# uber/fiber

Hardware: AMD Instinct MI355X
Metric: es_rollouts_per_sec (higher is better)
Workload: dtype bf16; 1 GPU; model=es-mlp-obs4-h64x64-act2, global_batch=2097152, seq_len=256, parallelism=dp1, pop_per_gpu=32768, envs_per_member=64

## Files before the change

### fiber_amd/csrc/ops/bindings.cpp

```cpp

#include <hip/hip_bf16.h>
#include <hip/hip_runtime.h>
#include <pybind11/pybind11.h>
#include <rocprim/rocprim.hpp>

#include <stdexcept>
#include <string>

namespace py = pybind11;

#define NPARAMS_HOST 4610
#define ENVS_HOST 64
#define OBS_HOST 4

extern "C" __global__ void es_rollout_mlp(
    const float*, float, uint32_t, uint32_t, int, int, const float*,
    const float*, const float*, const float*, float*, float*, float*);
extern "C" __global__ void es_eval_matrix(const float*, const float*,
                                          const float*, const float*,
                                          const float*, uint32_t, uint32_t,
                                          int, int, float*, float*);
extern "C" __global__ void obs_stat_reduce(const float*, int, float*);
extern "C" __global__ void es_grad(const float*, int, int, int, uint32_t,
                                   uint32_t, int, float*);
extern "C" __global__ void es_grad_reduce(const float*, int, int, float*);
extern "C" __global__ void centered_rank(const float*, int, float*);
extern "C" __global__ void rank_pack_keys(const float*, int, unsigned*,
                                          unsigned*);
extern "C" __global__ void rank_scatter(const unsigned*, int, float*);
extern "C" __global__ void mlp_policy_forward(const float*, const float*,
                                              int, float*);
extern "C" __global__ void mfma_gemm64_probe(const float*, const float*,
                                             float*);
extern "C" __global__ void es_perturb(const float*, int, int, float,
                                      uint32_t, const uint32_t*, int,
                                      __hip_bfloat16*, unsigned char*,
                                      unsigned char*);
extern "C" __global__ void conv_env_init(uint32_t, const uint32_t*, int,
                                         float*, float*);
extern "C" __global__ void conv_noisegen(uint32_t, const uint32_t*,
                                         uint32_t, unsigned char*);
extern "C" __global__ void conv_layer1(const __hip_bfloat16*,
                                       const unsigned char*, const float*,
                                       const __hip_bfloat16*,
                                       const unsigned char*, int,
                                       __hip_bfloat16*);
extern "C" __global__ void conv_layer2(const __hip_bfloat16*,
                                       const __hip_bfloat16*, int,
                                       unsigned char*);
extern "C" __global__ void conv_fc(const __hip_bfloat16*,
                                   const unsigned char*,
                                   const unsigned char*, int,
                                   __hip_bfloat16*);
extern "C" __global__ void conv_head_env(const __hip_bfloat16*,
                                         const __hip_bfloat16*, int,
                                         const float*, const float*, float*,
                                         float*);

static void check(hipError_t err, const char* what) {
  if (err != hipSuccess) {
    throw std::runtime_error(std::string(what) + ": " +
                             hipGetErrorString(err));
  }
}

static void launch_rollout(uintptr_t theta, double sigma, uint32_t seed,
                           uint32_t iter, int horizon, int member_offset,
                           int pop_shard, uintptr_t obs_mu, uintptr_t obs_nu,
                           uintptr_t env_A, uintptr_t env_B,
                           uintptr_t fitness, uintptr_t obs_stat_part,
                           uintptr_t obs_stat, uintptr_t stream) {
  if (pop_shard <= 0) return;
  hipLaunchKernelGGL(es_rollout_mlp, dim3(pop_shard), dim3(256), 0,
                     (hipStream_t)stream, (const float*)theta, (float)sigma,
                     seed, iter, horizon, member_offset,
                     (const float*)obs_mu, (const float*)obs_nu,
                     (const float*)env_A, (const float*)env_B,
                     (float*)fitness, (float*)obs_stat_part,
                     (float*)obs_stat);
  check(hipGetLastError(), "es_rollout_mlp launch");
  hipLaunchKernelGGL(obs_stat_reduce, dim3(2 * OBS_HOST), dim3(256), 0,
                     (hipStream_t)stream, (const float*)obs_stat_part,
                     pop_shard, (float*)obs_stat);
  check(hipGetLastError(), "obs_stat_reduce launch");
}

static void launch_eval_matrix(uintptr_t thetas, uintptr_t obs_mu,
                               uintptr_t obs_nu, uintptr_t env_A,
                               uintptr_t env_B, uint32_t seed, uint32_t iter,
                               int horizon, int K, int M, uintptr_t scores,
                               uintptr_t episodes, uintptr_t stream) {
  if (K <= 0 || M <= 0) return;
  const long long cells = (long long)K * (long long)M;
  if (cells > 0x7FFFFFFFLL)
    throw std::runtime_error("es_eval_matrix: K*M exceeds the grid limit");
  if (horizon < 1)
    throw std::runtime_error("es_eval_matrix: horizon must be >= 1");
  hipLaunchKernelGGL(es_eval_matrix, dim3((unsigned)cells), dim3(256), 0,
                     (hipStream_t)stream, (const float*)thetas,
                     (const float*)obs_mu, (const float*)obs_nu,
                     (const float*)env_A, (const float*)env_B, seed, iter,
                     horizon, M, (float*)scores, (float*)episodes);
  check(hipGetLastError(), "es_eval_matrix launch");
}

static int grad_chunks(int pairs, int nparams) {
  const int bx = ((nparams + 3) / 4 + 255) / 256;
  return pairs < 64 ? 1 : (bx >= 32 ? 4 : 32);
}

static void launch_grad(uintptr_t wpair, int pair_begin, int pair_end,
                        uint32_t seed, uint32_t iter, int nparams,
                        uintptr_t grad_part, uintptr_t grad,
                        uintptr_t stream) {
  const int jblocks = (nparams + 3) / 4;
  const int bx = (jblocks + 255) / 256;
  int pairs = pair_end - pair_begin;
  if (pairs <= 0) return;
  const int chunks = grad_chunks(pairs, nparams);
  int per_chunk = (pairs + chunks - 1) / chunks;
  hipLaunchKernelGGL(es_grad, dim3(bx, chunks), dim3(256), 0,
                     (hipStream_t)stream, (const float*)wpair, pair_begin,
                     pair_end, per_chunk, seed, iter, nparams,
                     chunks == 1 ? (float*)grad : (float*)grad_part);
  check(hipGetLastError(), "es_grad launch");
  if (chunks > 1) {
    hipLaunchKernelGGL(es_grad_reduce, dim3((nparams + 255) / 256),
                       dim3(256), 0, (hipStream_t)stream,
                       (const float*)grad_part, chunks, nparams,
                       (float*)grad);
    check(hipGetLastError(), "es_grad_reduce launch");
  }
}

static void launch_centered_rank(uintptr_t f, int n, uintptr_t out,
                                 uintptr_t stream) {
  const int bx = (n + 255) / 256;
  hipLaunchKernelGGL(centered_rank, dim3(bx), dim3(256), 0,
                     (hipStream_t)stream, (const float*)f, n, (float*)out);
  check(hipGetLastError(), "centered_rank launch");
}

static inline uint64_t rank_array_stride(int n) {
  return (((uint64_t)n * 4) + 255) & ~(uint64_t)255;
}

static uint64_t centered_rank_sorted_workspace(int n) {
  size_t temp_bytes = 0;
  check(rocprim::radix_sort_pairs(nullptr, temp_bytes,
                                  (const unsigned*)nullptr,
                                  (unsigned*)nullptr,
                                  (const unsigned*)nullptr,
                                  (unsigned*)nullptr, (size_t)n),
        "radix_sort_pairs size query");
  return 4 * rank_array_stride(n) + (uint64_t)temp_bytes + 256;
}

static void launch_centered_rank_sorted(uintptr_t f, int n, uintptr_t out,
                                        uintptr_t work, uint64_t work_bytes,
                                        uintptr_t stream) {
  const uint64_t stride = rank_array_stride(n);
  if (work_bytes < 4 * stride)
    throw std::runtime_error("centered_rank_sorted workspace too small");
  unsigned* keys_in = (unsigned*)work;
  unsigned* keys_out = (unsigned*)(work + stride);
  unsigned* vals_in = (unsigned*)(work + 2 * stride);
  unsigned* vals_out = (unsigned*)(work + 3 * stride);
  void* temp = (void*)(work + 4 * stride);
  size_t temp_bytes = (size_t)(work_bytes - 4 * stride);
  const int bx = (n + 255) / 256;
  hipLaunchKernelGGL(rank_pack_keys, dim3(bx), dim3(256), 0,
                     (hipStream_t)stream, (const float*)f, n, keys_in,
                     vals_in);
  check(hipGetLastError(), "rank_pack_keys launch");
  check(rocprim::radix_sort_pairs(temp, temp_bytes, keys_in, keys_out,
                                  vals_in, vals_out, (size_t)n, 0, 32,
                                  (hipStream_t)stream),
        "radix_sort_pairs");
  hipLaunchKernelGGL(rank_scatter, dim3(bx), dim3(256), 0,
                     (hipStream_t)stream, vals_out, n, (float*)out);
  check(hipGetLastError(), "rank_scatter launch");
}

static void launch_mlp_forward(uintptr_t theta, uintptr_t x, int batch,
                               uintptr_t logits, uintptr_t stream) {
  const int bx = (batch + ENVS_HOST - 1) / ENVS_HOST;
  hipLaunchKernelGGL(mlp_policy_forward, dim3(bx), dim3(256), 0,
                     (hipStream_t)stream, (const float*)theta,
                     (const float*)x, batch, (float*)logits);
  check(hipGetLastError(), "mlp_policy_forward launch");
}

static void launch_gemm64_probe(uintptr_t a, uintptr_t b, uintptr_t c,
                                uintptr_t stream) {
  hipLaunchKernelGGL(mfma_gemm64_probe, dim3(1), dim3(256), 0,
                     (hipStream_t)stream, (const float*)a, (const float*)b,
                     (float*)c);
  check(hipGetLastError(), "mfma_gemm64_probe launch");
}


static void launch_perturb(uintptr_t theta, int nparams, int np_pad,
                           double sigma, uint32_t seed, uintptr_t iterp,
                           int member_offset, int pop, uintptr_t wpert,
                           uintptr_t w3_fp8, uintptr_t w1_fp8,
                           uintptr_t stream) {
  if ((member_offset | pop) & 1)
    throw std::runtime_error(
        "es_perturb needs pair-aligned member_offset/pop");
  const int bx = 64;
  hipLaunchKernelGGL(es_perturb, dim3(bx, pop / 2), dim3(256), 0,
                     (hipStream_t)stream, (const float*)theta, nparams,
                     np_pad, (float)sigma, seed, (const uint32_t*)iterp,
                     member_offset, (__hip_bfloat16*)wpert,
                     (unsigned char*)w3_fp8, (unsigned char*)w1_fp8);
  check(hipGetLastError(), "es_perturb launch");
}

static void launch_conv_env_init(uint32_t seed, uintptr_t iterp,
                                 int nmembers, uintptr_t state,
                                 uintptr_t racc, uintptr_t stream) {
  const int n = nmembers * 16;
  hipLaunchKernelGGL(conv_env_init, dim3((n + 255) / 256), dim3(256), 0,
                     (hipStream_t)stream, seed, (const uint32_t*)iterp,
                     nmembers, (float*)state, (float*)racc);
  check(hipGetLastError(), "conv_env_init launch");
}

static void launch_conv_noisegen(uint32_t seed, uintptr_t iterp, uint32_t t,
                                 int nenv, uintptr_t znoise,
                                 uintptr_t stream) {
  const int total = nenv * (84 * 84 / 4);
  hipLaunchKernelGGL(conv_noisegen, dim3((total + 255) / 256), dim3(256), 0,
                     (hipStream_t)stream, seed, (const uint32_t*)iterp, t,
                     (unsigned char*)znoise);
  check(hipGetLastError(), "conv_noisegen launch");
}

static void launch_conv_layer1(uintptr_t wpert, uintptr_t w1_fp8,
                               uintptr_t state, uintptr_t gtab,
                               uintptr_t znoise, uintptr_t act1,
                               int nmembers, uintptr_t stream) {
  const int nenv = nmembers * 16;
  hipLaunchKernelGGL(conv_layer1, dim3(nenv), dim3(256), 0,
                     (hipStream_t)stream, (const __hip_bfloat16*)wpert,
                     (const unsigned char*)w1_fp8, (const float*)state,
                     (const __hip_bfloat16*)gtab,
                     (const unsigned char*)znoise, nenv,
                     (__hip_bfloat16*)act1);
  check(hipGetLastError(), "conv_layer1 launch");
}

static void launch_conv_layer2(uintptr_t wpert, uintptr_t act1,
                               uintptr_t act2, int nmembers,
                               uintptr_t stream) {
  const int nenv = nmembers * 16;
  hipLaunchKernelGGL(conv_layer2, dim3(nenv), dim3(256), 0,
                     (hipStream_t)stream, (const __hip_bfloat16*)wpert,
                     (const __hip_bfloat16*)act1, nenv,
                     (unsigned char*)act2);
  check(hipGetLastError(), "conv_layer2 launch");
}

static void launch_conv_fc(uintptr_t wpert, uintptr_t w3_fp8,
                           uintptr_t act2, uintptr_t act3, int nmembers,
                           uintptr_t stream) {
  hipLaunchKernelGGL(conv_fc, dim3(nmembers, 4), dim3(256), 0,
                     (hipStream_t)stream, (const __hip_bfloat16*)wpert,
                     (const unsigned char*)w3_fp8,
                     (const unsigned char*)act2, nmembers,
                     (__hip_bfloat16*)act3);
  check(hipGetLastError(), "conv_fc launch");
}

static void launch_conv_forward(uintptr_t wpert, uintptr_t w3_fp8,
                                uintptr_t w1_fp8, uintptr_t state,
                                uintptr_t gtab, uintptr_t znoise,
                                uintptr_t act1, uintptr_t act2,
                                uintptr_t act3, int nmembers,
                                uintptr_t stream) {
  launch_conv_layer1(wpert, w1_fp8, state, gtab, znoise, act1, nmembers,
                     stream);
  launch_conv_layer2(wpert, act1, act2, nmembers, stream);
  launch_conv_fc(wpert, w3_fp8, act2, act3, nmembers, stream);
}

static void launch_conv_head_env(uintptr_t wpert, uintptr_t act3,
                                 int nmembers, uintptr_t env_A,
                                 uintptr_t env_B, uintptr_t state,
                                 uintptr_t racc, uintptr_t stream) {
  hipLaunchKernelGGL(conv_head_env, dim3(nmembers), dim3(256), 0,
                     (hipStream_t)stream, (const __hip_bfloat16*)wpert,
                     (const __hip_bfloat16*)act3, nmembers,
                     (const float*)env_A, (const float*)env_B,
                     (float*)state, (float*)racc);
  check(hipGetLastError(), "conv_head_env launch");
}

PYBIND11_MODULE(_ops, m) {
  m.doc() = "fiber_amd CDNA4 ES kernels (gfx950)";
  m.attr("NPARAMS") = NPARAMS_HOST;
  m.attr("ENVS_PER_MEMBER") = ENVS_HOST;
  m.def("es_rollout_mlp", &launch_rollout, py::arg("theta"),
        py::arg("sigma"), py::arg("seed"), py::arg("iter"),
        py::arg("horizon"), py::arg("member_offset"), py::arg("pop_shard"),
        py::arg("obs_mu"), py::arg("obs_nu"), py::arg("env_A"),
        py::arg("env_B"), py::arg("fitness"), py::arg("obs_stat_part"),
        py::arg("obs_stat"), py::arg("stream"));
  m.def("es_eval_matrix", &launch_eval_matrix, py::arg("thetas"),
        py::arg("obs_mu"), py::arg("obs_nu"), py::arg("env_A"),
        py::arg("env_B"), py::arg("seed"), py::arg("iter"),
        py::arg("horizon"), py::arg("K"), py::arg("M"), py::arg("scores"),
        py::arg("episodes"), py::arg("stream"));
  m.def("es_grad", &launch_grad, py::arg("wpair"), py::arg("pair_begin"),
        py::arg("pair_end"), py::arg("seed"), py::arg("iter"),
        py::arg("nparams"), py::arg("grad_part"), py::arg("grad"),
        py::arg("stream"));
  m.def("es_grad_chunks", &grad_chunks, py::arg("pairs"),
        py::arg("nparams"));
  m.def("centered_rank", &launch_centered_rank, py::arg("f"), py::arg("n"),
        py::arg("out"), py::arg("stream"));
  m.def("centered_rank_sorted_workspace", &centered_rank_sorted_workspace,
        py::arg("n"));
  m.def("centered_rank_sorted", &launch_centered_rank_sorted, py::arg("f"),
        py::arg("n"), py::arg("out"), py::arg("work"),
        py::arg("work_bytes"), py::arg("stream"));
  m.def("mlp_policy_forward", &launch_mlp_forward, py::arg("theta"),
        py::arg("x"), py::arg("batch"), py::arg("logits"),
        py::arg("stream"));
  m.def("mfma_gemm64_probe", &launch_gemm64_probe, py::arg("a"),
        py::arg("b"), py::arg("c"), py::arg("stream"));

  m.attr("NP_CONV") = 677686;
  m.attr("NP_CONV_PAD") = 677688;
  m.attr("CONV_ENVS") = 16;
  m.def("es_perturb", &launch_perturb, py::arg("theta"), py::arg("nparams"),
        py::arg("np_pad"), py::arg("sigma"), py::arg("seed"),
        py::arg("iterp"), py::arg("member_offset"), py::arg("pop"),
        py::arg("wpert"), py::arg("w3_fp8"), py::arg("w1_fp8"),
        py::arg("stream"));
  m.def("conv_env_init", &launch_conv_env_init, py::arg("seed"),
        py::arg("iterp"), py::arg("nmembers"), py::arg("state"),
        py::arg("racc"), py::arg("stream"));
  m.def("conv_noisegen", &launch_conv_noisegen, py::arg("seed"),
        py::arg("iterp"), py::arg("t"), py::arg("nenv"),
        py::arg("znoise"), py::arg("stream"));
  m.def("conv_forward", &launch_conv_forward, py::arg("wpert"),
        py::arg("w3_fp8"), py::arg("w1_fp8"), py::arg("state"),
        py::arg("gtab"), py::arg("znoise"), py::arg("act1"),
        py::arg("act2"), py::arg("act3"), py::arg("nmembers"),
        py::arg("stream"));
  m.def("conv_layer1", &launch_conv_layer1, py::arg("wpert"),
        py::arg("w1_fp8"), py::arg("state"), py::arg("gtab"),
        py::arg("znoise"), py::arg("act1"), py::arg("nmembers"),
        py::arg("stream"));
  m.def("conv_layer2", &launch_conv_layer2, py::arg("wpert"),
        py::arg("act1"), py::arg("act2"), py::arg("nmembers"),
        py::arg("stream"));
  m.def("conv_fc", &launch_conv_fc, py::arg("wpert"), py::arg("w3_fp8"),
        py::arg("act2"), py::arg("act3"), py::arg("nmembers"),
        py::arg("stream"));
  m.def("conv_head_env", &launch_conv_head_env, py::arg("wpert"),
        py::arg("act3"), py::arg("nmembers"), py::arg("env_A"),
        py::arg("env_B"), py::arg("state"), py::arg("racc"),
        py::arg("stream"));
}
```

### fiber_amd/csrc/ops/es_kernels.hip

```cpp

#include <hip/hip_bf16.h>
#include <hip/hip_runtime.h>

#include "philox.h"

typedef __attribute__((ext_vector_type(8))) __bf16 bf16x8;
typedef __attribute__((ext_vector_type(4))) float f32x4;
typedef __attribute__((ext_vector_type(2))) float f32x2;

#define TWO_LOG2E 0x1.715476p+1f
__device__ inline float fast_tanh(float x) {
  float e = __builtin_amdgcn_exp2f(x * TWO_LOG2E);
  return 1.0f - 2.0f * __builtin_amdgcn_rcpf(e + 1.0f);
}

__device__ inline f32x2 tanh2_bias(f32x2 acc, f32x2 bias) {
  const f32x2 m = (acc + bias) * TWO_LOG2E;
  f32x2 e;
  e.x = __builtin_amdgcn_exp2f(m.x);
  e.y = __builtin_amdgcn_exp2f(m.y);
  const f32x2 ep1 = e + 1.0f;
  f32x2 r;
  r.x = __builtin_amdgcn_rcpf(ep1.x);
  r.y = __builtin_amdgcn_rcpf(ep1.y);
  return __builtin_elementwise_fma(r, (f32x2){-2.0f, -2.0f},
                                   (f32x2){1.0f, 1.0f});
}

__device__ inline f32x4 fast_tanh4_bias(f32x4 acc, f32x4 bias) {
  const f32x2 lo = tanh2_bias(acc.lo, bias.lo);
  const f32x2 hi = tanh2_bias(acc.hi, bias.hi);
  return __builtin_shufflevector(lo, hi, 0, 1, 2, 3);
}

#define FAM_TAG_NOISE 0x45530001u
#define FAM_TAG_ENV 0x45530002u

#define OBS 4
#define KPAD 32
#define HID 64
#define ACT 2
#define ENVS 64

#define OFF_W1 0
#define OFF_B1 (HID * OBS)
#define OFF_W2 (OFF_B1 + HID)
#define OFF_B2 (OFF_W2 + HID * HID)
#define OFF_W3 (OFF_B2 + HID)
#define OFF_B3 (OFF_W3 + ACT * HID)
#define NPARAMS (OFF_B3 + ACT)

#define S1 8
#define S2 72

template <int S, bool NARROW>
__device__ inline const bf16x8* strip_frag_ptr(
    const __hip_bfloat16* __restrict__ M, const __hip_bfloat16* zero16,
    int row, int kk, int kgrp) {
  if (NARROW)
    return reinterpret_cast<const bf16x8*>(kgrp == 0 ? &M[row * S] : zero16);
  return reinterpret_cast<const bf16x8*>(&M[row * S + kk * 32 + kgrp * 8]);
}

template <int K, int AS, bool NARROW = false>
__device__ inline void strip_load_a(const __hip_bfloat16* __restrict__ A,
                                    const __hip_bfloat16* zero16, int wave,
                                    int lane, bf16x8 (&afrag)[K / 32]) {
#pragma unroll
  for (int kk = 0; kk < K / 32; ++kk)
    afrag[kk] = *strip_frag_ptr<AS, NARROW>(A, zero16,
                                            wave * 16 + (lane & 15), kk,
                                            lane >> 4);
}

__device__ inline f32x4 strip_load_bias(const float* __restrict__ bias,
                                        int wave, int lane) {
  return *reinterpret_cast<const f32x4*>(
      &bias[wave * 16 + (lane >> 4) * 4]);
}

template <int K, int BS, bool NARROW>
__device__ inline f32x4 strip_mfma(const bf16x8 (&afrag)[K / 32],
                                   const __hip_bfloat16* __restrict__ B,
                                   const __hip_bfloat16* zero16, int ct,
                                   int lane) {
  f32x4 acc = {0.f, 0.f, 0.f, 0.f};
#pragma unroll
  for (int kk = 0; kk < K / 32; ++kk) {
    const bf16x8 bfrag = *strip_frag_ptr<BS, NARROW>(
        B, zero16, ct * 16 + (lane & 15), kk, lane >> 4);
    acc = __builtin_amdgcn_mfma_f32_16x16x32_bf16(afrag[kk], bfrag, acc, 0,
                                                  0, 0);
  }
  return acc;
}

template <int K, int BS, int OS, bool NARROW = false>
__device__ inline void mfma_strip_tanh_pre(
    const bf16x8 (&afrag)[K / 32], const __hip_bfloat16* __restrict__ B,
    const __hip_bfloat16* zero16, f32x4 biasq,
    __hip_bfloat16* __restrict__ out, int wave, int lane) {
#pragma unroll
  for (int ct = 0; ct < 4; ++ct) {
    const int bcol = ct * 16 + (lane & 15);
    const f32x4 acc = strip_mfma<K, BS, NARROW>(afrag, B, zero16, ct, lane);
    const int drow = wave * 16 + (lane >> 4) * 4;
    const f32x4 th = fast_tanh4_bias(acc, biasq);
    union {
      __hip_bfloat16 h[4];
      unsigned long long u;
    } pk;
#pragma unroll
    for (int ri = 0; ri < 4; ++ri) pk.h[ri] = __float2bfloat16(th[ri]);
    *reinterpret_cast<unsigned long long*>(&out[bcol * OS + drow]) = pk.u;
  }
}

template <int K, int AS, int BS, int OS, bool NARROW = false>
__device__ inline void mfma_strip_tanh(const __hip_bfloat16* __restrict__ A,
                                       const __hip_bfloat16* __restrict__ B,
                                       const float* __restrict__ bias,
                                       __hip_bfloat16* __restrict__ out,
                                       int wave, int lane,
                                       const __hip_bfloat16* zero16 = nullptr) {
  bf16x8 afrag[K / 32];
  strip_load_a<K, AS, NARROW>(A, zero16, wave, lane, afrag);
  mfma_strip_tanh_pre<K, BS, OS, NARROW>(
      afrag, B, zero16, strip_load_bias(bias, wave, lane), out, wave, lane);
}

template <int K, int BS>
__device__ inline void mfma_strip_logits(
    const bf16x8 (&afrag)[K / 32], const __hip_bfloat16* __restrict__ B,
    f32x4 biasq, const float* __restrict__ w3r, float (*lpart)[ENVS][2],
    int wave, int lane) {
#pragma unroll
  for (int ct = 0; ct < 4; ++ct) {
    const f32x4 acc = strip_mfma<K, BS, false>(afrag, B, nullptr, ct, lane);
    const f32x4 h = fast_tanh4_bias(acc, biasq);
    float p0 = 0.f, p1 = 0.f;
#pragma unroll
    for (int ri = 0; ri < 4; ++ri) {
      p0 += w3r[ri] * h[ri];
      p1 += w3r[4 + ri] * h[ri];
    }
    p0 += __shfl_xor(p0, 16, 64);
    p1 += __shfl_xor(p1, 16, 64);
    p0 += __shfl_xor(p0, 32, 64);
    p1 += __shfl_xor(p1, 32, 64);
    if ((lane >> 4) == 0) {
      lpart[wave][ct * 16 + lane][0] = p0;
      lpart[wave][ct * 16 + lane][1] = p1;
    }
  }
}

struct PolicyLds {
  alignas(16) __hip_bfloat16 w1[HID][S1];
  alignas(16) __hip_bfloat16 w2[HID][S2];
  alignas(16) __hip_bfloat16 w3[ACT][HID];
  alignas(16) float b1[HID];
  alignas(16) float b2[HID];
  float b3[ACT];
};

__device__ inline void store_param(PolicyLds* p, int j, float v) {
  if (j < OFF_B1) {
    p->w1[j >> 2][j & 3] = __float2bfloat16(v);
  } else if (j < OFF_W2) {
    p->b1[j - OFF_B1] = v;
  } else if (j < OFF_B2) {
    int jj = j - OFF_W2;
    p->w2[jj >> 6][jj & 63] = __float2bfloat16(v);
  } else if (j < OFF_W3) {
    p->b2[j - OFF_B2] = v;
  } else if (j < OFF_B3) {
    int jj = j - OFF_W3;
    p->w3[jj >> 6][jj & 63] = __float2bfloat16(v);
  } else if (j < NPARAMS) {
    p->b3[j - OFF_B3] = v;
  }
}

struct RolloutLds {
  PolicyLds pol;
  alignas(16) __hip_bfloat16 xb[ENVS][S1];
  alignas(16) __hip_bfloat16 zero16[8];
  alignas(16) __hip_bfloat16 h1[ENVS][S2];
  float S[2][ENVS][OBS];
  float lpart[4][ENVS][2];
  float ostat[2 * OBS + 1];
};


template <bool STATS>
__device__ __forceinline__ void rollout_init_lds(RolloutLds& L, int tid,
                                                 uint32_t seed,
                                                 uint32_t iter) {
  for (int idx = tid; idx < HID * (S1 - OBS); idx += blockDim.x) {
    L.pol.w1[idx / (S1 - OBS)][OBS + idx % (S1 - OBS)] =
        __float2bfloat16(0.f);
  }
  for (int idx = tid; idx < ENVS * (S1 - OBS); idx += blockDim.x) {
    L.xb[idx / (S1 - OBS)][OBS + idx % (S1 - OBS)] =
        __float2bfloat16(0.f);
  }
  if (tid < 8) L.zero16[tid] = __float2bfloat16(0.f);
  if (tid < ENVS) {
    float z[4];
    fam_normal4(seed, iter, (uint32_t)tid, 0u, FAM_TAG_ENV, 0u, z);
#pragma unroll
    for (int d = 0; d < OBS; ++d) L.S[0][tid][d] = 0.3f * z[d];
  }
  if (STATS) {
    if (tid < 2 * OBS + 1) L.ostat[tid] = 0.f;
  }
}

template <bool STATS>
__device__ __forceinline__ float rollout_steps(
    RolloutLds& L, int tid, int horizon, const float* obs_mu,
    const float* obs_nu,
    const float* env_A,
    const float* env_B,
    float& psum, float& psq) {
  const int lane = tid & 63;
  const int wave = tid >> 6;
  const int env = tid & 63;
  const int dd = tid >> 6;
  float raccp = 0.f;
  const float mu_d = obs_mu[dd];
  const float rstd_d = rsqrtf(obs_nu[dd] + 1e-4f);
  float eA_d[OBS];
#pragma unroll
  for (int e = 0; e < OBS; ++e) eA_d[e] = env_A[dd * OBS + e];
  const float eB_d = env_B[dd];
  const float one_if_d0 = (dd == 0) ? 1.f : 0.f;
  float w3r[2 * 4];
  {
    const int drow = wave * 16 + (lane >> 4) * 4;
#pragma unroll
    for (int ri = 0; ri < 4; ++ri) {
      w3r[ri] = __bfloat162float(L.pol.w3[0][drow + ri]);
      w3r[4 + ri] = __bfloat162float(L.pol.w3[1][drow + ri]);
    }
  }

  bf16x8 a1[KPAD / 32], a2[HID / 32];
  strip_load_a<KPAD, S1, true>(&L.pol.w1[0][0], L.zero16, wave, lane, a1);
  strip_load_a<HID, S2>(&L.pol.w2[0][0], nullptr, wave, lane, a2);
  const f32x4 b1q = strip_load_bias(L.pol.b1, wave, lane);
  const f32x4 b2q = strip_load_bias(L.pol.b2, wave, lane);

  {
    const float s = L.S[0][env][dd];
    if (STATS) {
      psum += s;
      psq += s * s;
    }
    float x = (s - mu_d) * rstd_d;
    L.xb[env][dd] = __float2bfloat16(fminf(5.f, fmaxf(-5.f, x)));
  }

  for (int t = 0; t < horizon; ++t) {
    const int cur = t & 1;
    __syncthreads();
    mfma_strip_tanh_pre<KPAD, S1, S2, true>(a1, &L.xb[0][0], L.zero16, b1q,
                                            &L.h1[0][0], wave, lane);
    __syncthreads();
    mfma_strip_logits<HID, S2>(a2, &L.h1[0][0], b2q, w3r, L.lpart, wave,
                               lane);
    __syncthreads();
    {
      const float l0 = L.pol.b3[0] + L.lpart[0][env][0] +
                       L.lpart[1][env][0] + L.lpart[2][env][0] +
                       L.lpart[3][env][0];
      const float l1 = L.pol.b3[1] + L.lpart[0][env][1] +
                       L.lpart[1][env][1] + L.lpart[2][env][1] +
                       L.lpart[3][env][1];
      const float asign = (l1 > l0) ? 1.f : -1.f;
      float drive = 0.f;
#pragma unroll
      for (int e = 0; e < OBS; ++e) drive += eA_d[e] * L.S[cur][env][e];
      const float snew =
          fmaf(0.08f, fast_tanh(drive), 0.97f * L.S[cur][env][dd]) +
          0.05f * eB_d * asign;
      L.S[cur ^ 1][env][dd] = snew;
      raccp += one_if_d0 - 0.1f * snew * snew;
      if (t < horizon - 1) {
        if (STATS) {
          psum += snew;
          psq += snew * snew;
        }
        float x = (snew - mu_d) * rstd_d;
        L.xb[env][dd] = __float2bfloat16(fminf(5.f, fmaxf(-5.f, x)));
      }
    }
  }
  __syncthreads();
  return raccp;
}

__device__ __forceinline__ float reward_reduce_wave0(
    const RolloutLds& L, int lane, float* __restrict__ episodes) {
  float r = L.lpart[0][lane][0] + L.lpart[1][lane][0] +
            L.lpart[2][lane][0] + L.lpart[3][lane][0];
  if (episodes != nullptr) episodes[lane] = r;
#pragma unroll
  for (int off = 32; off > 0; off >>= 1) r += __shfl_down(r, off, 64);
  return r;
}

extern "C" __global__ void __launch_bounds__(256)
es_rollout_mlp(const float* __restrict__ theta, float sigma, uint32_t seed,
               uint32_t iter, int horizon, int member_offset,
               const float* __restrict__ obs_mu,
               const float* __restrict__ obs_nu,
               const float* __restrict__ env_A,
               const float* __restrict__ env_B,
               float* __restrict__ fitness,
               float* __restrict__ obs_stat_part,
               float* __restrict__ obs_stat_out)
{
  __shared__ RolloutLds L;
  const int tid = threadIdx.x;
  const int lane = tid & 63;
  const int wave = tid >> 6;
  const int member = member_offset + blockIdx.x;
  const uint32_t pair = (uint32_t)(member >> 1);
  const float sgn = (member & 1) ? -sigma : sigma;

  for (int jb = tid; jb * 4 < NPARAMS; jb += blockDim.x) {
    float z[4];
    fam_normal4(seed, iter, pair, (uint32_t)jb, FAM_TAG_NOISE, 0u, z);
    const int j0 = jb * 4;
#pragma unroll
    for (int u = 0; u < 4; ++u) {
      const int j = j0 + u;
      if (j < NPARAMS) store_param(&L.pol, j, theta[j] + sgn * z[u]);
    }
  }
  rollout_init_lds<true>(L, tid, seed, iter);
  __syncthreads();

  const int env = tid & 63;
  const int dd = tid >> 6;
  float psum = 0.f, psq = 0.f;
  const float raccp = rollout_steps<true>(L, tid, horizon, obs_mu, obs_nu,
                                          env_A, env_B, psum, psq);

  L.lpart[dd][env][0] = raccp;
#pragma unroll
  for (int off = 32; off > 0; off >>= 1) {
    psum += __shfl_down(psum, off, 64);
    psq += __shfl_down(psq, off, 64);
  }
  if (lane == 0) {
    L.ostat[dd] = psum;
    L.ostat[OBS + dd] = psq;
  }
  __syncthreads();
  if (wave == 0) {
    const float r = reward_reduce_wave0(L, lane, nullptr);
    if (lane == 0) fitness[blockIdx.x] = r / (float)ENVS;
  }
  if (tid < 2 * OBS)
    obs_stat_part[(size_t)blockIdx.x * (2 * OBS) + tid] = L.ostat[tid];
  if (tid == 0)
    atomicAdd(&obs_stat_out[2 * OBS], (float)(ENVS * horizon));
}

extern "C" __global__ void __launch_bounds__(256)
es_eval_matrix(const float* __restrict__ thetas,
               const float* __restrict__ obs_mu,
               const float* __restrict__ obs_nu,
               const float* __restrict__ env_A,
               const float* __restrict__ env_B,
               uint32_t seed, uint32_t iter, int horizon, int M,
               float* __restrict__ scores,
               float* __restrict__ episodes)
{
  __shared__ RolloutLds L;
  const int tid = threadIdx.x;
  const size_t cell = blockIdx.x;
  const size_t k = cell / (size_t)M;
  const size_t m = cell % (size_t)M;

  const float* __restrict__ theta = thetas + k * NPARAMS;
  for (int j = tid; j < NPARAMS; j += blockDim.x)
    store_param(&L.pol, j, theta[j]);
  rollout_init_lds<false>(L, tid, seed, iter);
  __syncthreads();

  float psum = 0.f, psq = 0.f;
  const float raccp = rollout_steps<false>(
      L, tid, horizon, obs_mu + k * OBS, obs_nu + k * OBS,
      env_A + m * (OBS * OBS), env_B + m * OBS, psum, psq);

  L.lpart[tid >> 6][tid & 63][0] = raccp;
  __syncthreads();
  if (tid < 64) {
    const float r = reward_reduce_wave0(
        L, tid, episodes != nullptr ? episodes + cell * ENVS : nullptr);
    if (tid == 0) scores[cell] = r / (float)ENVS;
  }
}

extern "C" __global__ void __launch_bounds__(256)
obs_stat_reduce(const float* __restrict__ part, int nmembers,
                float* __restrict__ obs_stat_out) {
  __shared__ float red[256];
  const int tid = threadIdx.x;
  const int col = blockIdx.x;
  float acc = 0.f;
  for (int m = tid; m < nmembers; m += 256)
    acc += part[(size_t)m * (2 * OBS) + col];
  red[tid] = acc;
  __syncthreads();
  for (int s = 128; s > 0; s >>= 1) {
    if (tid < s) red[tid] += red[tid + s];
    __syncthreads();
  }
  if (tid == 0) obs_stat_out[col] = red[0];
}

extern "C" __global__ void es_grad(const float* __restrict__ wpair,
                                   int pair_begin, int pair_end,
                                   int pairs_per_chunk, uint32_t seed,
                                   uint32_t iter, int nparams,
                                   float* __restrict__ out) {
  const int jb = blockIdx.x * blockDim.x + threadIdx.x;
  if (jb * 4 >= nparams) return;
  const int chunk_begin = pair_begin + blockIdx.y * pairs_per_chunk;
  const int chunk_end = min(chunk_begin + pairs_per_chunk, pair_end);
  float acc[4] = {0.f, 0.f, 0.f, 0.f};
  for (int pair = chunk_begin; pair < chunk_end; ++pair) {
    const float w = wpair[pair];
    if (w == 0.f) continue;
    float z[4];
    fam_normal4(seed, iter, (uint32_t)pair, (uint32_t)jb, FAM_TAG_NOISE, 0u,
                z);
#pragma unroll
    for (int u = 0; u < 4; ++u) acc[u] += w * z[u];
  }
  float* __restrict__ row = out + (size_t)blockIdx.y * nparams;
#pragma unroll
  for (int u = 0; u < 4; ++u) {
    const int j = jb * 4 + u;
    if (j < nparams) row[j] = acc[u];
  }
}

extern "C" __global__ void es_grad_reduce(const float* __restrict__ part,
                                          int chunks, int nparams,
                                          float* __restrict__ grad) {
  const int j = blockIdx.x * blockDim.x + threadIdx.x;
  if (j >= nparams) return;
  float acc = 0.f;
  for (int c = 0; c < chunks; ++c) acc += part[(size_t)c * nparams + j];
  grad[j] = acc;
}

extern "C" __global__ void centered_rank(const float* __restrict__ f, int n,
                                         float* __restrict__ out) {
  const int i = blockIdx.x * blockDim.x + threadIdx.x;
  if (i >= n) return;
  const float fi = f[i];
  int rank = 0;
  for (int j = 0; j < n; ++j) {
    const float fj = f[j];
    rank += (fj < fi) || (fj == fi && j < i);
  }
  out[i] = (float)rank / (float)(n - 1) - 0.5f;
}

extern "C" __global__ void rank_pack_keys(const float* __restrict__ f, int n,
                                          unsigned* __restrict__ keys,
                                          unsigned* __restrict__ vals) {
  const int i = blockIdx.x * blockDim.x + threadIdx.x;
  if (i >= n) return;
  unsigned u = __float_as_uint(f[i]);
  if ((u & 0x7FFFFFFFu) == 0u) u = 0u;
  keys[i] = (u & 0x80000000u) ? ~u : (u | 0x80000000u);
  vals[i] = (unsigned)i;
}

extern "C" __global__ void rank_scatter(const unsigned* __restrict__ vals,
                                        int n, float* __restrict__ out) {
  const int k = blockIdx.x * blockDim.x + threadIdx.x;
  if (k >= n) return;
  out[vals[k]] = (float)k / (float)(n - 1) - 0.5f;
}

extern "C" __global__ void __launch_bounds__(256)
mlp_policy_forward(const float* __restrict__ theta,
                   const float* __restrict__ X, int batch,
                   float* __restrict__ logits) {
  __shared__ PolicyLds pol;
  __shared__ alignas(16) __hip_bfloat16 xb[ENVS][S1];
  __shared__ alignas(16) __hip_bfloat16 zero16[8];
  __shared__ alignas(16) __hip_bfloat16 h1[ENVS][S2];
  __shared__ alignas(16) __hip_bfloat16 h2[ENVS][S2];
  const int tid = threadIdx.x;
  const int lane = tid & 63;
  const int wave = tid >> 6;
  const int row0 = blockIdx.x * ENVS;

  for (int j = tid; j < NPARAMS; j += blockDim.x) store_param(&pol, j, theta[j]);
  for (int idx = tid; idx < HID * (S1 - OBS); idx += blockDim.x)
    pol.w1[idx / (S1 - OBS)][OBS + idx % (S1 - OBS)] =
        __float2bfloat16(0.f);
  for (int idx = tid; idx < ENVS * S1; idx += blockDim.x) {
    int e = idx / S1, d = idx % S1;
    float v = (d < OBS && row0 + e < batch) ? X[(row0 + e) * OBS + d] : 0.f;
    xb[e][d] = __float2bfloat16(v);
  }
  if (tid < 8) zero16[tid] = __float2bfloat16(0.f);
  __syncthreads();
  mfma_strip_tanh<KPAD, S1, S1, S2, true>(&pol.w1[0][0], &xb[0][0], pol.b1,
                                          &h1[0][0], wave, lane, zero16);
  __syncthreads();
  mfma_strip_tanh<HID, S2, S2, S2>(&pol.w2[0][0], &h1[0][0], pol.b2,
                                   &h2[0][0], wave, lane);
  __syncthreads();
  if (tid < ENVS && row0 + tid < batch) {
#pragma unroll
    for (int a = 0; a < ACT; ++a) {
      float l = pol.b3[a];
      for (int h = 0; h < HID; ++h)
        l += __bfloat162float(pol.w3[a][h]) *
             __bfloat162float(h2[tid][h]);
      logits[(row0 + tid) * ACT + a] = l;
    }
  }
}

extern "C" __global__ void __launch_bounds__(256)
mfma_gemm64_probe(const float* __restrict__ A64,
                  const float* __restrict__ B64,
                  float* __restrict__ C64T) {
  __shared__ alignas(16) __hip_bfloat16 a[HID][S2];
  __shared__ alignas(16) __hip_bfloat16 b[HID][S2];
  __shared__ alignas(16) __hip_bfloat16 c[HID][S2];
  __shared__ alignas(16) float zero_bias[HID];
  const int tid = threadIdx.x;
  for (int idx = tid; idx < HID * HID; idx += blockDim.x) {
    int r = idx >> 6, k = idx & 63;
    a[r][k] = __float2bfloat16(A64[r * HID + k]);
    b[r][k] = __float2bfloat16(B64[k * HID + r]);
  }
  if (tid < HID) zero_bias[tid] = 0.f;
  __syncthreads();
  mfma_strip_tanh<HID, S2, S2, S2>(&a[0][0], &b[0][0], zero_bias, &c[0][0],
                                   tid >> 6, tid & 63);
  __syncthreads();
  for (int idx = tid; idx < HID * HID; idx += blockDim.x) {
    int col = idx >> 6, row = idx & 63;
    C64T[col * HID + row] = __bfloat162float(c[col][row]);
  }
}
```

### fiber_amd/ops/__init__.py

```python

import torch

_OPS = None
_IMPORT_ERROR = None

try:
    from fiber_amd import _ops as _OPS
except ImportError as exc:
    _IMPORT_ERROR = exc


NPARAMS = _OPS.NPARAMS if _OPS else 4610
ENVS_PER_MEMBER = _OPS.ENVS_PER_MEMBER if _OPS else 64
OBS_DIM = 4
ACT_DIM = 2
HIDDEN = 64


def _require_ops():
    if _OPS is None:
        raise RuntimeError(
            "fiber_amd._ops (gfx950 HIP extension) is not built: %r. "
            "Run `python setup.py build_ext --inplace` "
            "(PYTORCH_ROCM_ARCH=gfx950)." % (_IMPORT_ERROR,)
        )
    return _OPS


def _stream():
    return torch.cuda.current_stream().cuda_stream


def _check(t, name, dtype=torch.float32, device=True):
    if t.dtype != dtype:
        raise TypeError("%s must be %s, got %s" % (name, dtype, t.dtype))
    if device and not t.is_cuda:
        raise TypeError("%s must be a CUDA (ROCm) tensor" % name)
    if not t.is_contiguous():
        raise TypeError("%s must be contiguous" % name)
    return t


def _partial_buffer(device, numel):
    return torch.empty(numel, dtype=torch.float32, device=device)


def es_rollout_mlp(theta, sigma, seed, iteration, horizon, member_offset,
                   pop_shard, obs_mu, obs_nu, env_A, env_B):
    ops = _require_ops()
    _check(theta, "theta")
    assert theta.numel() == NPARAMS
    fitness = torch.empty(pop_shard, dtype=torch.float32,
                          device=theta.device)
    obs_stat = torch.zeros(2 * OBS_DIM + 1, dtype=torch.float32,
                           device=theta.device)
    part = _partial_buffer(theta.device, int(pop_shard) * 2 * OBS_DIM)
    ops.es_rollout_mlp(
        theta.data_ptr(), float(sigma), int(seed) & 0xFFFFFFFF,
        int(iteration) & 0xFFFFFFFF, int(horizon), int(member_offset),
        int(pop_shard), _check(obs_mu, "obs_mu").data_ptr(),
        _check(obs_nu, "obs_nu").data_ptr(),
        _check(env_A, "env_A").data_ptr(),
        _check(env_B, "env_B").data_ptr(), fitness.data_ptr(),
        part.data_ptr(), obs_stat.data_ptr(), _stream())
    return fitness, obs_stat


def es_eval_matrix(thetas, obs_mu, obs_nu, env_A, env_B, seed, iteration,
                   horizon, return_episodes=False):
    ops = _require_ops()
    named = (("thetas", thetas), ("obs_mu", obs_mu), ("obs_nu", obs_nu),
             ("env_A", env_A), ("env_B", env_B))
    for name, t in named:
        _check(t, name)
        if t.device != thetas.device:
            raise TypeError("%s is on %s, thetas on %s"
                            % (name, t.device, thetas.device))
    if thetas.dim() != 2 or thetas.shape[1] != NPARAMS:
        raise ValueError("thetas must be [K, %d], got %s"
                         % (NPARAMS, tuple(thetas.shape)))
    K = thetas.shape[0]
    if env_A.dim() != 3 or tuple(env_A.shape[1:]) != (OBS_DIM, OBS_DIM):
        raise ValueError("env_A must be [M, %d, %d], got %s"
                         % (OBS_DIM, OBS_DIM, tuple(env_A.shape)))
    M = env_A.shape[0]
    for name, t, want in (("obs_mu", obs_mu, (K, OBS_DIM)),
                          ("obs_nu", obs_nu, (K, OBS_DIM)),
                          ("env_B", env_B, (M, OBS_DIM))):
        if tuple(t.shape) != want:
            raise ValueError("%s must be %s, got %s"
                             % (name, list(want), tuple(t.shape)))
    horizon = int(horizon)
    if horizon < 1:
        raise ValueError("horizon must be >= 1, got %d" % horizon)
    if K * M >= 2 ** 31:
        raise ValueError("K*M = %d exceeds the launch grid" % (K * M))
    device = thetas.device
    scores = torch.empty(K, M, dtype=torch.float32, device=device)
    episodes = None
    if return_episodes:
        episodes = torch.empty(K, M, ENVS_PER_MEMBER, dtype=torch.float32,
                               device=device)
    with torch.cuda.device(device):
        ops.es_eval_matrix(
            thetas.data_ptr(), obs_mu.data_ptr(), obs_nu.data_ptr(),
            env_A.data_ptr(), env_B.data_ptr(), int(seed) & 0xFFFFFFFF,
            int(iteration) & 0xFFFFFFFF, horizon, K, M, scores.data_ptr(),
            episodes.data_ptr() if return_episodes else 0, _stream())
    if return_episodes:
        return scores, episodes
    return scores


def es_grad(wpair, pair_begin, pair_end, seed, iteration, device,
            nparams=None):
    ops = _require_ops()
    _check(wpair, "wpair")
    if nparams is None:
        nparams = NPARAMS
    grad = torch.zeros(nparams, dtype=torch.float32, device=device)
    chunks = ops.es_grad_chunks(int(pair_end) - int(pair_begin),
                                int(nparams))
    part = _partial_buffer(grad.device, chunks * int(nparams))
    ops.es_grad(wpair.data_ptr(), int(pair_begin), int(pair_end),
                int(seed) & 0xFFFFFFFF, int(iteration) & 0xFFFFFFFF,
                int(nparams), part.data_ptr(), grad.data_ptr(), _stream())
    return grad


_rank_workspace = {}


def centered_rank(fitness):
    _check(fitness, "fitness")
    n = fitness.numel()
    ops = _require_ops()
    out = torch.empty_like(fitness)
    if n > 16384:
        dev = fitness.device
        cached = _rank_workspace.get(dev)
        if cached is None or cached[0] < n:
            need = ops.centered_rank_sorted_workspace(n)
            cached = (n, torch.empty(need, dtype=torch.uint8, device=dev))
            _rank_workspace[dev] = cached
        ws = cached[1]
        ops.centered_rank_sorted(fitness.data_ptr(), n, out.data_ptr(),
                                 ws.data_ptr(), ws.numel(), _stream())
        return out
    ops.centered_rank(fitness.data_ptr(), n, out.data_ptr(), _stream())
    return out


def centered_rank_ref(fitness):
    n = fitness.numel()
    order = torch.argsort(torch.argsort(fitness, stable=True))
    return order.float() / (n - 1) - 0.5


def mlp_policy_forward(theta, x):
    ops = _require_ops()
    _check(theta, "theta")
    _check(x, "x")
    batch = x.shape[0]
    logits = torch.empty(batch, ACT_DIM, dtype=torch.float32,
                         device=x.device)
    ops.mlp_policy_forward(theta.data_ptr(), x.data_ptr(), batch,
                           logits.data_ptr(), _stream())
    return logits


def mlp_policy_forward_ref(theta, x):
    w1 = theta[:256].view(HIDDEN, OBS_DIM)
    b1 = theta[256:320]
    w2 = theta[320:4416].view(HIDDEN, HIDDEN)
    b2 = theta[4416:4480]
    w3 = theta[4480:4608].view(ACT_DIM, HIDDEN)
    b3 = theta[4608:4610]
    bf = lambda t: t.to(torch.bfloat16).to(torch.float32)
    h1 = torch.tanh(bf(x) @ bf(w1).T + b1)
    h2 = torch.tanh(bf(h1) @ bf(w2).T + b2)
    return bf(h2) @ bf(w3).T + b3


def mfma_gemm64_probe(a, b):
    ops = _require_ops()
    _check(a, "a")
    _check(b, "b")
    out_t = torch.empty(64, 64, dtype=torch.float32, device=a.device)
    ops.mfma_gemm64_probe(a.data_ptr(), b.data_ptr(), out_t.data_ptr(),
                          _stream())
    return out_t.T.contiguous()


def ops_available():
    return _OPS is not None
```

Measured before the change: 108.4 million rollouts/s.

## Alias h1 onto W2 LDS tile, use permlane swaps for logits, raise occupancy

Replaces the per-column-tile shfl_xor reduction of logit partials with permlane16/permlane32 swap instructions that reduce two column tiles at once and write all four k-groups' results. Removes the separate h1 LDS buffer by aliasing it onto the W2 tile. Adds a minimum-waves hint of 7 to the rollout and eval kernels' launch bounds. The LDS saving and the launch-bound hint aim to fit more workgroups per CU, at the cost of register-pressure limits. Aliasing h1 onto W2 is only safe if W2 is no longer read from LDS once h1 is written. A probe kernel is added to check that the two reductions agree.

```diff
diff --git a/fiber_amd/csrc/ops/bindings.cpp b/fiber_amd/csrc/ops/bindings.cpp
--- a/fiber_amd/csrc/ops/bindings.cpp
+++ b/fiber_amd/csrc/ops/bindings.cpp
@@ -32,6 +32,8 @@
                                               int, float*);
 extern "C" __global__ void mfma_gemm64_probe(const float*, const float*,
                                              float*);
+extern "C" __global__ void logits_reduce_probe(const float*, const float*,
+                                               float*, float*);
 extern "C" __global__ void es_perturb(const float*, int, int, float,
                                       uint32_t, const uint32_t*, int,
                                       __hip_bfloat16*, unsigned char*,
@@ -199,6 +201,16 @@
   check(hipGetLastError(), "mfma_gemm64_probe launch");
 }
 
+static void launch_logits_reduce_probe(uintptr_t p0, uintptr_t p1,
+                                       uintptr_t out_shfl,
+                                       uintptr_t out_swap,
+                                       uintptr_t stream) {
+  hipLaunchKernelGGL(logits_reduce_probe, dim3(1), dim3(64), 0,
+                     (hipStream_t)stream, (const float*)p0,
+                     (const float*)p1, (float*)out_shfl, (float*)out_swap);
+  check(hipGetLastError(), "logits_reduce_probe launch");
+}
+
 
 static void launch_perturb(uintptr_t theta, int nparams, int np_pad,
                            double sigma, uint32_t seed, uintptr_t iterp,
@@ -330,6 +342,9 @@
         py::arg("stream"));
   m.def("mfma_gemm64_probe", &launch_gemm64_probe, py::arg("a"),
         py::arg("b"), py::arg("c"), py::arg("stream"));
+  m.def("logits_reduce_probe", &launch_logits_reduce_probe, py::arg("p0"),
+        py::arg("p1"), py::arg("out_shfl"), py::arg("out_swap"),
+        py::arg("stream"));
 
   m.attr("NP_CONV") = 677686;
   m.attr("NP_CONV_PAD") = 677688;
diff --git a/fiber_amd/csrc/ops/es_kernels.hip b/fiber_amd/csrc/ops/es_kernels.hip
--- a/fiber_amd/csrc/ops/es_kernels.hip
+++ b/fiber_amd/csrc/ops/es_kernels.hip
@@ -129,29 +129,64 @@
       afrag, B, zero16, strip_load_bias(bias, wave, lane), out, wave, lane);
 }
 
+__device__ inline void logits_reduce_shfl(float p0, float p1,
+                                          float (*lrow)[2], int ct,
+                                          int lane) {
+  p0 += __shfl_xor(p0, 16, 64);
+  p1 += __shfl_xor(p1, 16, 64);
+  p0 += __shfl_xor(p0, 32, 64);
+  p1 += __shfl_xor(p1, 32, 64);
+  if ((lane >> 4) == 0) {
+    lrow[ct * 16 + lane][0] = p0;
+    lrow[ct * 16 + lane][1] = p1;
+  }
+}
+
+__device__ inline f32x2 permlane16_swap(float x, float y) {
+  const auto r = __builtin_amdgcn_permlane16_swap(
+      __float_as_uint(x), __float_as_uint(y), false, false);
+  return (f32x2){__uint_as_float(r[0]), __uint_as_float(r[1])};
+}
+
+__device__ inline f32x2 permlane32_swap(float x, float y) {
+  const auto r = __builtin_amdgcn_permlane32_swap(
+      __float_as_uint(x), __float_as_uint(y), false, false);
+  return (f32x2){__uint_as_float(r[0]), __uint_as_float(r[1])};
+}
+
+__device__ inline void logits_reduce_swap(float p0a, float p1a, float p0b,
+                                          float p1b, float (*lrow)[2],
+                                          int ct, int lane) {
+  const f32x2 sa = permlane16_swap(p0a, p1a);
+  const f32x2 sb = permlane16_swap(p0b, p1b);
+  const f32x2 s = permlane32_swap(sa.x + sa.y, sb.x + sb.y);
+  const int kgrp = lane >> 4;
+  lrow[(ct + (kgrp >> 1)) * 16 + (lane & 15)][kgrp & 1] = s.x + s.y;
+}
+
 template <int K, int BS>
 __device__ inline void mfma_strip_logits(
     const bf16x8 (&afrag)[K / 32], const __hip_bfloat16* __restrict__ B,
-    f32x4 biasq, const float* __restrict__ w3r, float (*lpart)[ENVS][2],
-    int wave, int lane) {
-#pragma unroll
-  for (int ct = 0; ct < 4; ++ct) {
-    const f32x4 acc = strip_mfma<K, BS, false>(afrag, B, nullptr, ct, lane);
-    const f32x4 h = fast_tanh4_bias(acc, biasq);
-    float p0 = 0.f, p1 = 0.f;
-#pragma unroll
-    for (int ri = 0; ri < 4; ++ri) {
-      p0 += w3r[ri] * h[ri];
-      p1 += w3r[4 + ri] * h[ri];
+    f32x4 biasq, const f32x2 (&w3p)[4], float (*lpart)[ENVS][2], int wave,
+    int lane) {
+#pragma unroll
+  for (int cp = 0; cp < 4; cp += 2) {
+    f32x2 p[2];
+#pragma unroll
+    for (int c = 0; c < 2; ++c) {
+      const f32x4 acc =
+          strip_mfma<K, BS, false>(afrag, B, nullptr, cp + c, lane);
+      const f32x4 h = fast_tanh4_bias(acc, biasq);
+      float p0 = 0.f, p1 = 0.f;
+#pragma unroll
+      for (int ri = 0; ri < 4; ++ri) {
+        p0 += w3p[ri].x * h[ri];
+        p1 += w3p[ri].y * h[ri];
+      }
+      p[c] = (f32x2){p0, p1};
     }
-    p0 += __shfl_xor(p0, 16, 64);
-    p1 += __shfl_xor(p1, 16, 64);
-    p0 += __shfl_xor(p0, 32, 64);
-    p1 += __shfl_xor(p1, 32, 64);
-    if ((lane >> 4) == 0) {
-      lpart[wave][ct * 16 + lane][0] = p0;
-      lpart[wave][ct * 16 + lane][1] = p1;
-    }
+    logits_reduce_swap(p[0].x, p[0].y, p[1].x, p[1].y, lpart[wave], cp,
+                       lane);
   }
 }
 
@@ -186,11 +221,13 @@
   PolicyLds pol;
   alignas(16) __hip_bfloat16 xb[ENVS][S1];
   alignas(16) __hip_bfloat16 zero16[8];
-  alignas(16) __hip_bfloat16 h1[ENVS][S2];
   float S[2][ENVS][OBS];
   float lpart[4][ENVS][2];
   float ostat[2 * OBS + 1];
+
+  __device__ __hip_bfloat16* h1() { return &pol.w2[0][0]; }
 };
+static_assert(ENVS == HID, "h1 [ENVS][S2] shares the W2 tile [HID][S2]");
 
 
 template <bool STATS>
@@ -236,13 +273,13 @@
   for (int e = 0; e < OBS; ++e) eA_d[e] = env_A[dd * OBS + e];
   const float eB_d = env_B[dd];
   const float one_if_d0 = (dd == 0) ? 1.f : 0.f;
-  float w3r[2 * 4];
+  f32x2 w3p[4];
   {
     const int drow = wave * 16 + (lane >> 4) * 4;
 #pragma unroll
     for (int ri = 0; ri < 4; ++ri) {
-      w3r[ri] = __bfloat162float(L.pol.w3[0][drow + ri]);
-      w3r[4 + ri] = __bfloat162float(L.pol.w3[1][drow + ri]);
+      w3p[ri].x = __bfloat162float(L.pol.w3[0][drow + ri]);
+      w3p[ri].y = __bfloat162float(L.pol.w3[1][drow + ri]);
     }
   }
 
@@ -266,10 +303,9 @@
     const int cur = t & 1;
     __syncthreads();
     mfma_strip_tanh_pre<KPAD, S1, S2, true>(a1, &L.xb[0][0], L.zero16, b1q,
-                                            &L.h1[0][0], wave, lane);
+                                            L.h1(), wave, lane);
     __syncthreads();
-    mfma_strip_logits<HID, S2>(a2, &L.h1[0][0], b2q, w3r, L.lpart, wave,
-                               lane);
+    mfma_strip_logits<HID, S2>(a2, L.h1(), b2q, w3p, L.lpart, wave, lane);
     __syncthreads();
     {
       const float l0 = L.pol.b3[0] + L.lpart[0][env][0] +
@@ -281,7 +317,8 @@
       const float asign = (l1 > l0) ? 1.f : -1.f;
       float drive = 0.f;
 #pragma unroll
-      for (int e = 0; e < OBS; ++e) drive += eA_d[e] * L.S[cur][env][e];
+      for (int e = 0; e < OBS; ++e)
+        drive = fmaf(eA_d[e], L.S[cur][env][e], drive);
       const float snew =
           fmaf(0.08f, fast_tanh(drive), 0.97f * L.S[cur][env][dd]) +
           0.05f * eB_d * asign;
@@ -311,7 +348,11 @@
   return r;
 }
 
-extern "C" __global__ void __launch_bounds__(256)
+#ifndef ROLLOUT_WAVES
+#define ROLLOUT_WAVES 7
+#endif
+
+extern "C" __global__ void __launch_bounds__(256, ROLLOUT_WAVES)
 es_rollout_mlp(const float* __restrict__ theta, float sigma, uint32_t seed,
                uint32_t iter, int horizon, int member_offset,
                const float* __restrict__ obs_mu,
@@ -370,7 +411,7 @@
     atomicAdd(&obs_stat_out[2 * OBS], (float)(ENVS * horizon));
 }
 
-extern "C" __global__ void __launch_bounds__(256)
+extern "C" __global__ void __launch_bounds__(256, ROLLOUT_WAVES)
 es_eval_matrix(const float* __restrict__ thetas,
                const float* __restrict__ obs_mu,
                const float* __restrict__ obs_nu,
@@ -559,3 +600,31 @@
     C64T[col * HID + row] = __bfloat162float(c[col][row]);
   }
 }
+
+extern "C" __global__ void __launch_bounds__(64)
+logits_reduce_probe(const float* __restrict__ p0,
+                    const float* __restrict__ p1,
+                    float* __restrict__ out_shfl,
+                    float* __restrict__ out_swap)
+{
+  __shared__ float lrow[2][ENVS][2];
+  const int lane = threadIdx.x;
+  float a[4], b[4];
+#pragma unroll
+  for (int ct = 0; ct < 4; ++ct) {
+    a[ct] = p0[ct * 64 + lane];
+    b[ct] = p1[ct * 64 + lane];
+  }
+#pragma unroll
+  for (int ct = 0; ct < 4; ++ct)
+    logits_reduce_shfl(a[ct], b[ct], lrow[0], ct, lane);
+#pragma unroll
+  for (int cp = 0; cp < 4; cp += 2)
+    logits_reduce_swap(a[cp], b[cp], a[cp + 1], b[cp + 1], lrow[1], cp, lane);
+  __syncthreads();
+#pragma unroll
+  for (int a01 = 0; a01 < 2; ++a01) {
+    out_shfl[lane * 2 + a01] = lrow[0][lane][a01];
+    out_swap[lane * 2 + a01] = lrow[1][lane][a01];
+  }
+}
diff --git a/fiber_amd/ops/__init__.py b/fiber_amd/ops/__init__.py
--- a/fiber_amd/ops/__init__.py
+++ b/fiber_amd/ops/__init__.py
@@ -192,5 +192,23 @@
     return out_t.T.contiguous()
 
 
+def logits_reduce_probe(p0, p1):
+    ops = _require_ops()
+    for name, t in (("p0", p0), ("p1", p1)):
+        _check(t, name)
+        if tuple(t.shape) != (4, 64):
+            raise ValueError("%s must be [4, 64], got %s"
+                             % (name, tuple(t.shape)))
+    if p1.device != p0.device:
+        raise TypeError("p1 is on %s, p0 on %s" % (p1.device, p0.device))
+    shfl = torch.empty(ENVS_PER_MEMBER, ACT_DIM, dtype=torch.float32,
+                       device=p0.device)
+    swap = torch.empty_like(shfl)
+    with torch.cuda.device(p0.device):
+        ops.logits_reduce_probe(p0.data_ptr(), p1.data_ptr(),
+                                shfl.data_ptr(), swap.data_ptr(), _stream())
+    return shfl, swap
+
+
 def ops_available():
     return _OPS is not None
```

Result: faster. 112.8 million rollouts/s (median of 6 runs) (+4.1%).
